# AndreiBarsan/DynSLAM

Measured on AMD Instinct MI355X. Metric: frames/sec TSDF integrate+raycast (KITTI 1242x375, 5mm voxels); HBM GB/s vs peak, higher is better.
Workload: dtype f32; 1 GPU; configs[1]: static map only, synthetic KITTI-like street 1242x375, preset 5mm (voxel 0.005 m, mu 0.02 m), frames 5..2062 of a 2063-frame sequence, one volume per GPU; visible_blocks_last_frame=122661, allocated_blocks=8388608, status=3, decay=False, swap=False, instances=0

## Files before the change

dynslam_amd/csrc/dsr_device.h:

```cpp
#pragma once
#include <hip/hip_runtime.h>
#include <stdint.h>

#include "../../include/dsr.h"

namespace dsr {

constexpr int kBlockSize = DSR_BLOCK_SIZE;
constexpr int kBlockSize3 = DSR_BLOCK_SIZE3;
constexpr int kBlockBytes = 4096;

constexpr int kOffSdf = 0;
constexpr int kOffWDepth = 1024;
constexpr int kOffClr = 2048;

constexpr float kFarAway = 999999.9f;
constexpr float kVeryClose = 0.05f;
constexpr int kMinmaxSubsample = 8;

enum Ctr {
  CTR_LAST_FREE_BLOCK = 0,
  CTR_LAST_FREE_EXCESS = 1,
  CTR_NO_VISIBLE_LIVE = 2,
  CTR_NO_VISIBLE_FREE = 3,
// ... 31 lines not shown
  Mat4 M_rgb;
  float4 proj;
  float4 proj_rgb;
  float mu, voxelSize;
  float vfMin, vfMax;
  int W, H, Wr, Hr;
  int maxW, stopAtMaxW, depthWeighting, rgbSame;
  int noBuckets, noExcess, noTotalEntries, noBlocks;
  uint32_t hashMask;
  uint32_t maxSteps;
  int useSwapping;
};

struct SceneP {
  dsr_hash_entry *table;
  uint8_t *vba;
  int32_t *voxelAllocList;
  int32_t *excessAllocList;
  int32_t *ctr;
  unsigned long long *work;
  uint32_t *allocKey;
  uint32_t *allocGrp;
  unsigned long long *allocTile;
  uint8_t *swapState;
  uint8_t *swapStored;
  int32_t *swapSlot;
  uint8_t **hostSlabs;
  int slabBlocks;
  uint8_t *visGrp;
  uint32_t *visBits;
  uint32_t *allocBits;
  int32_t *allocIds;
  float *icpPose;
};
constexpr int kIcpPoseWords = 20;
__device__ __forceinline__ void write_icp_pose(const SceneP &s, const Mat4 &M) {
  if (blockIdx.x == 0 && blockIdx.y == 0 && threadIdx.x < 17) s.icpPose[threadIdx.x] = threadIdx.x < 16 ? M.m[threadIdx.x] : 1.0f;
}


__device__ __forceinline__ int f2i(float f) {
  int r;
  asm("v_cvt_i32_f32 %0, %1" : "=v"(r) : "v"(f));
  return r;
}
__device__ __forceinline__ short f2s(float f) { return (short)f2i(f); }
// ... 68 lines not shown
template <int NT>
__device__ __forceinline__ int2 wg_exclusive_scan2(int2 v, int2 &total, int2 *lds) {
  const int lane = threadIdx.x & 63, wid = threadIdx.x >> 6;
  int2 inc = v;
#pragma unroll
  for (int d = 1; d < 64; d <<= 1) {
    int ox = __shfl_up(inc.x, d), oy = __shfl_up(inc.y, d);
    if (lane >= d) { inc.x += ox; inc.y += oy; }
  }
  if (lane == 63) lds[wid] = inc;
  __syncthreads();
  int2 woff = make_int2(0, 0), tot = make_int2(0, 0);
#pragma unroll
  for (int w = 0; w < NT / 64; ++w) {
    int2 s = lds[w];
    if (w < wid) { woff.x += s.x; woff.y += s.y; }
    tot.x += s.x; tot.y += s.y;
  }
  __syncthreads();
  total = tot;
  return make_int2(woff.x + inc.x - v.x, woff.y + inc.y - v.y);
}

constexpr int kTileThreads = 256;
constexpr int kTileItems = 8;
constexpr int kTile = kTileThreads * kTileItems;

}
```

dynslam_amd/csrc/dsr_engine.hip:

```cpp
#include <sched.h>

#include "dsr_internal.h"
#include "dsr_math.h"
using namespace dsr_internal;
#include "k_alloc.h"
#include "k_composite.h"
#include "k_decay.h"
#include "k_integrate.h"
#include "k_raycast.h"
#include "k_swap.h"
#include "k_mesh.h"
#include "k_small.h"
#include "k_batch.h"
#include "k_batch_gc.h"
#include "../../include/dsr_track.h"
#include "../../include/dsr_gc.h"

extern "C" {
int dsri_batch_flush(dsr_batch *b);
bool dsri_batch_is_live(dsr_batch *b);
void dsri_batch_drop_deferred(dsr_batch *b);
}

namespace dsr_internal {
// ... 67 lines not shown
}

int reset_scene(dsr_engine *e) {
  e->sceneVersion++;
  e->noVisibleValid = false;
  e->listVersion++;
  LAUNCH(e, "reset", k_reset_table, dim3(div_up(e->E, 256)), dim3(256), e->scene.table, e->E, e->scene.allocKey);
  LAUNCH(e, "reset", k_iota, dim3(div_up(e->noExcess, 256)), dim3(256), e->scene.excessAllocList, e->noExcess);
  LAUNCH(e, "reset", k_iota, dim3(div_up(e->noBlocks, 256)), dim3(256), e->scene.voxelAllocList, e->noBlocks);
  LAUNCH(e, "reset", k_reset_vba, dim3(4096), dim3(256), reinterpret_cast<uint4 *>(e->scene.vba),
         (size_t)e->noBlocks * (kBlockBytes / 16));
  LAUNCH(e, "reset", k_reset_counters, dim3(1), dim3(64), e->scene.ctr, e->scene.work, e->noBlocks, e->noExcess);
  if (e->scene.swapState) {
    HIP_TRY(hipMemsetAsync(e->scene.swapState, 0, (size_t)e->E, e->stream));
    HIP_TRY(hipMemsetAsync(e->scene.swapStored, 0, (size_t)e->E, e->stream));
    HIP_TRY(hipMemsetAsync(e->scene.swapSlot, 0xff, (size_t)e->E * 4, e->stream));
    HIP_TRY(hipStreamSynchronize(e->stream));
    e->hostUsedUpper = 0; e->hostUsedPending = false; e->hostUsedCallsSince = 0;
  }
  HIP_TRY(hipMemsetAsync(e->live.visType, 0, (size_t)e->E, e->stream));
  HIP_TRY(hipMemsetAsync(e->freeview.visType, 0, (size_t)e->E, e->stream));
  HIP_TRY(hipMemsetAsync(e->scene.allocGrp, 0, (size_t)e->numTilesE * (kTile / 32) * 4, e->stream));
  HIP_TRY(hipMemsetAsync(e->scene.allocTile, 0, ((size_t)e->numTilesE + 1) * 8, e->stream));
  if (e->scene.visBits) {
    HIP_TRY(hipMemsetAsync(e->scene.visGrp, 0, (size_t)kSmallBitWords * 4, e->stream));
    HIP_TRY(hipMemsetAsync(e->scene.visBits, 0, (size_t)kSmallBitWords * 4, e->stream));
    HIP_TRY(hipMemsetAsync(e->scene.allocBits, 0, (size_t)kSmallBitWords * 4, e->stream));
  }
  e->fifoHead = 0; e->fifoLen = 0;
  for (RenderStateDev *rs : {&e->live, &e->freeview})
    if (rs->rayBox) {
      hipLaunchKernelGGL(k_raybox_reset, dim3(1), dim3(RB_WORDS), 0, e->stream, rs->rayBox, (e->W + 7) / 8, (e->H + 7) / 8, e->rayBoxLive ? 1 : 0);
    }
  e->rayBoxLive = true;
  HIP_TRY(hipGetLastError());
  if (e->statusHost) {
    HIP_TRY(hipStreamSynchronize(e->stream));
    e->statusHost[0] = 0; e->statusHost[1] = DSR_OK;
  }
  return DSR_OK;
}

void free_all(dsr_engine *e) {
  auto F = [](void *p) { if (p) (void)hipFree(p); };
  F(e->scene.table); F(e->scene.vba); F(e->scene.voxelAllocList); F(e->scene.excessAllocList);
  F(e->scene.ctr); F(e->scene.icpPose); F(e->scene.work); F(e->scene.allocKey); F(e->scene.allocGrp); F(e->scene.allocTile);
  F(e->scene.visGrp); F(e->scene.visBits); F(e->scene.allocBits); F(e->scene.allocIds);
  for (RenderStateDev *rs : {&e->live, &e->freeview}) {
    F(rs->visibleIDs); F(rs->visibleIDsAlt); F(rs->visBlocks); F(rs->visBlocksAlt); F(rs->visType); F(rs->minmax); F(rs->raycastResult); F(rs->raycastImage); F(rs->rayBox);
  }
  dsr_internal::tracker_free(e);
  F(e->tileSums); F(e->integrateStats); F(e->allocList); F(e->allocWork); F(e->meshTris); F(e->rgb); F(e->depth); F(e->depthTmp); F(e->rawDepth); F(e->pointsMap); F(e->normalsMap);
  F(e->freeDepth); F(e->aosScratch);
  F(e->fifoPlanes); F(e->decayCand); F(e->decayFlags);
  if (e->maskHost) (void)hipHostFree(e->maskHost);
  for (auto ev : e->maskEvent) if (ev) (void)hipEventDestroy(ev);
  F(e->scene.swapState); F(e->scene.swapStored); F(e->swapStagingDev); F(e->swapIdsDev); F(e->swapFlagsDev);
  F(e->scene.swapSlot); F(e->scene.hostSlabs);
  if (e->hostUsedSeen) (void)hipHostFree(e->hostUsedSeen);
  if (e->hostUsedEvent) (void)hipEventDestroy(e->hostUsedEvent);
  for (auto p : e->hostSlabs) (void)hipHostFree(p);
  for (int k = 0; k < 2; ++k) {
    if (e->upPin[k]) (void)hipHostFree(e->upPin[k]);
    if (e->upSlotFree[k]) (void)hipEventDestroy(e->upSlotFree[k]);
  }
  F(e->upDev); F(e->pvDev); F(e->xferRgb); F(e->xferDepth);
  F(e->rgbAlt); F(e->depthAlt);
  for (hipEvent_t ev : {e->evAltFree, e->evFusionRead}) if (ev) (void)hipEventDestroy(ev);
  if (e->viewStream && e->ownsViewStream) (void)hipStreamDestroy(e->viewStream);
  if (e->pvPin) (void)hipHostFree(e->pvPin);
  if (e->statusHost) (void)hipHostFree(e->statusHost);
  for (hipEvent_t ev : {e->evUploaded, e->evIngested, e->evView, e->evViewRead}) if (ev) (void)hipEventDestroy(ev);
  if (e->xEvent) (void)hipEventDestroy(e->xEvent);
  if (e->xEvent2) (void)hipEventDestroy(e->xEvent2);
  if (e->orderEvent) (void)hipEventDestroy(e->orderEvent);
// ... 17 lines not shown
  { int st = before_fusion(e); if (st) return st; }
  if (e->sidePending) { HIP_TRY(hipStreamWaitEvent(e->stream, e->evExpected, 0)); e->sidePending = false; }
  if (e->smallPath) {
    const int tx0 = e->viewBox[0] / 16, ty0 = e->viewBox[1] / 16;
    const int tx1 = div_up(std::min(e->viewBox[2], e->W), 16), ty1 = div_up(std::min(e->viewBox[3], e->H), 16);
    if (tx1 > tx0 && ty1 > ty0)
      LAUNCH(e, "alloc_mark", k_alloc_mark<true>, dim3(tx1 - tx0, ty1 - ty0), dim3(256), p, e->scene, (const float *)e->depth,
             rs.visType, tx0, ty0);
    if (e->statusDev) e->statusSeq++;
    {
      ProfScope _ps(e, "small_alloc_visible");
      hipLaunchKernelGGL(k_small_alloc_visible, dim3(1), dim3(kSmallThreads), e->smallLdsBytes, e->stream, p, e->scene,
                         (const float *)e->depth, rs.visType, e->numTilesE, e->allocWork, rs.visibleIDs, rs.visBlocks, e->noBlocks,
                         e->statusDev, e->statusSeq, reinterpret_cast<int2 *>(rs.minmax), rs.rayBox, e->smallLists ? 1 : 0);
    }
    HIP_TRY(hipGetLastError());
    { int st = after_fusion(e); if (st) return st; }
    e->liveExp.valid = true; e->liveExp.onSide = false; e->liveExp.version = e->listVersion; e->liveExp.M = e->M_d;
    memcpy(e->liveExp.proj, proj, sizeof proj);
    return DSR_OK;
  }
  LAUNCH(e, "retest_prev_visible", k_retest_previous_visible, dim3(1024), dim3(256), p, e->scene,
         (const int4 *)rs.visBlocks, rs.visType);
  int2 *allocTile = reinterpret_cast<int2 *>(e->scene.allocTile);
  LAUNCH(e, "alloc_mark", k_alloc_mark<false>, dim3(div_up(e->W, 16), div_up(e->H, 16)), dim3(256), p, e->scene,
         (const float *)e->depth, rs.visType, 0, 0);
  LAUNCH(e, "scan_tiles", k_scan_tile_sums, dim3(1), dim3(1024), allocTile, e->numTilesE, e->scene, (int)SCAN_ALLOC, 0);
  LAUNCH(e, "alloc_commit", k_alloc_commit, dim3(e->numTilesE), dim3(kTileThreads), p, e->scene, allocTile, e->allocWork);
  LAUNCH(e, "alloc_apply", k_alloc_apply, dim3(256), dim3(256), p, e->scene, (const float *)e->depth,
         (const int4 *)e->allocWork, rs.visType);
  LAUNCH(e, "visible_count", k_visible_count<false>, dim3(e->numTilesE), dim3(kTileThreads), p, e->scene, rs.visType, e->tileSums);
  LAUNCH(e, "scan_tiles", k_scan_tile_sums, dim3(1), dim3(1024), e->tileSums, e->numTilesE, e->scene,
         (int)SCAN_VISIBLE_LIVE, e->noBlocks);
  if (e->statusDev) e->statusSeq++;
  LAUNCH(e, "visible_write", k_visible_write, dim3(e->numTilesE), dim3(kTileThreads), e->E, (const uint8_t *)rs.visType,
         (const int2 *)e->tileSums, rs.visibleIDs, e->noBlocks, e->scene, (int)e->s.use_swapping, rs.visBlocks, e->statusDev,
         e->statusSeq);
  HIP_TRY(hipGetLastError());
  { int st = after_fusion(e); if (st) return st; }
  e->liveExp.valid = false;
  if (e->overlapExpected && (e->device >= 64 || g_enginesOnDevice[e->device].load(std::memory_order_relaxed) <= 1)) {
    HIP_TRY(hipEventRecord(e->evList, e->stream));
    HIP_TRY(hipStreamWaitEvent(e->sideStream, e->evList, 0));
    {
      StreamSwap sw(e, e->sideStream);
      int st = expected_depths(e, rs, p);
      if (st) return st;
    }
    HIP_TRY(hipEventRecord(e->evExpected, e->sideStream));
    e->sidePending = true;
    e->liveExp.valid = true; e->liveExp.onSide = true; e->liveExp.version = e->listVersion; e->liveExp.M = e->M_d;
    memcpy(e->liveExp.proj, proj, sizeof proj);
  }
  return DSR_OK;
}

int integrate_scene(dsr_engine *e) {
  e->sceneVersion++;
  float proj[4]; depth_proj(e, proj);
  FrameP p = make_frame_params(e, e->M_d, e->invM_d, proj);
// ... 270 lines not shown
    if (e->device < 0 || e->device >= 64) return nullptr;
    std::lock_guard<std::mutex> lock(g_ioMutex);
    if (!table[e->device] && create_stream(&table[e->device]) != hipSuccess) table[e->device] = nullptr;
    return table[e->device];
  };
  if (pvMode == 3 && s.sdf_local_block_num <= 16384 && (e->stream = shared_stream(g_sharedViewStream))) e->ownsStream = false;
  else if (pvMode >= 2 && s.sdf_local_block_num <= 16384 && (e->stream = shared_stream(g_sharedSmallStream))) e->ownsStream = false;
  else if (create_stream(&e->stream) != hipSuccess) { delete e; return fail(DSR_E_DEVICE, "hipStreamCreate failed"); }
  e->overlapExpected = s.sdf_local_block_num >= (1 << 20);
  if (const char *ov = getenv("DSR_OVERLAP_EXPECTED")) e->overlapExpected = atoi(ov) != 0;
  if (e->overlapExpected &&
      (hipStreamCreateWithFlags(&e->sideStream, hipStreamNonBlocking) != hipSuccess ||
       hipEventCreateWithFlags(&e->evList, order_event_flags()) != hipSuccess ||
       hipEventCreateWithFlags(&e->evExpected, order_event_flags()) != hipSuccess)) { free_all(e); delete e; return fail(DSR_E_DEVICE, "side stream creation failed"); }
  ALLOC(dmalloc(&e->scene.table, (size_t)e->E));
  ALLOC(dmalloc(&e->scene.vba, (size_t)e->noBlocks * kBlockBytes));
  ALLOC(dmalloc(&e->scene.voxelAllocList, (size_t)e->noBlocks));
  ALLOC(dmalloc(&e->scene.excessAllocList, (size_t)e->noExcess));
  ALLOC(dmalloc(&e->scene.ctr, (size_t)CTR_COUNT));
  ALLOC(dmalloc(&e->scene.work, (size_t)WORK_COUNT));
  ALLOC(dmalloc(&e->scene.allocKey, (size_t)e->E));
  ALLOC(dmalloc(&e->scene.allocGrp, (size_t)e->numTilesE * (kTile / 32)));
  ALLOC(dmalloc(&e->scene.allocTile, (size_t)e->numTilesE + 1));
  {
    const int cells = ((e->W + 7) / 8) * ((e->H + 7) / 8);
    e->smallPath = e->smallVolume && !s.use_swapping && e->E <= kSmallMaxEntries && e->E % 8 == 0 && e->numTilesE <= kSmallMaxTiles &&
                   small_lds_bytes(cells) <= 64 * 1024;
    if (e->smallPath) {
      ALLOC(dmalloc(&e->scene.visGrp, (size_t)kSmallBitWords * 4));
      ALLOC(dmalloc(&e->scene.visBits, (size_t)kSmallBitWords));
      ALLOC(dmalloc(&e->scene.allocBits, (size_t)kSmallBitWords));
      ALLOC(dmalloc(&e->scene.allocIds, (size_t)e->noBlocks));
      e->smallLdsBytes = small_lds_bytes(cells);
      const size_t withLists = std::max(e->smallLdsBytes, sizeof(SmallShared) + small_lists_lds_bytes(e->noBlocks));
      e->smallLists = withLists <= 64 * 1024 && !(getenv("DSR_SMALL_LISTS") && atoi(getenv("DSR_SMALL_LISTS")) == 0);
      if (e->smallLists) e->smallLdsBytes = withLists;
      e->pairRender = pair_render_default();
    }
  }
  ALLOC(dmalloc(&e->allocWork, (size_t)std::min((double)e->noBlocks, (double)e->P * e->maxSteps)));
  const int mw = (e->W + 7) / 8, mh = (e->H + 7) / 8;
  for (RenderStateDev *rs : {&e->live, &e->freeview}) {
    ALLOC(dmalloc(&rs->visibleIDs, (size_t)e->noBlocks));
    ALLOC(dmalloc(&rs->visBlocks, (size_t)e->noBlocks));
    ALLOC(dmalloc(&rs->visType, (size_t)e->E));
    ALLOC(dmalloc(&rs->minmax, (size_t)mw * mh));
// ... 390 lines not shown
        break;
      }
      if (!cached && e->smallPath) {
        const int cells = ((e->W + 7) / 8) * ((e->H + 7) / 8);
        {
          ProfScope _ps(e, "small_freeview");
          hipLaunchKernelGGL(k_small_freeview, dim3(1), dim3(kSmallThreads), small_lds_bytes(cells), e->stream, p, e->scene, e->allocList,
                             rs.visibleIDs, rs.visBlocks, e->noBlocks, reinterpret_cast<int2 *>(rs.minmax), rs.rayBox, e->smallLists ? 1 : 0);
        }
        e->fvValid = true; e->fvVersion = e->sceneVersion; e->fvM = M; memcpy(e->fvProj, proj, sizeof proj);
        if (outIsDevice) {
          LAUNCH(e, "raycast_freeview", k_raycast_render, g, dim3(256), p, e->scene, (const float2 *)rs.minmax,
                 rs.raycastResult, type, rs.raycastImage, (float *)depth_out, (uchar4 *)rgba_out, rs.rayBox);
          HIP_TRY(hipGetLastError());
          break;
        }
        LAUNCH(e, "raycast_freeview", k_raycast_render, g, dim3(256), p, e->scene, (const float2 *)rs.minmax,
               rs.raycastResult, type, rs.raycastImage, depth_out ? e->freeDepth : (float *)nullptr, (uchar4 *)nullptr, rs.rayBox);
        HIP_TRY(hipGetLastError());
        if (rgba_out) HIP_TRY(hipMemcpyAsync(rgba_out, rs.raycastImage, P * 4, kind, e->stream));
        if (depth_out) HIP_TRY(hipMemcpyAsync(depth_out, e->freeDepth, P * 4, kind, e->stream));
        break;
      } else if (!cached && e->smallVolume) {
        LAUNCH(e, "freeview_visible", k_visible_count<true>, dim3(e->numTilesE), dim3(kTileThreads), p, e->scene, rs.visType, e->tileSums);
        LAUNCH(e, "scan_tiles", k_scan_tile_sums, dim3(1), dim3(1024), e->tileSums, e->numTilesE, e->scene,
               (int)SCAN_VISIBLE_FREE, e->noBlocks);
        LAUNCH(e, "freeview_visible", k_visible_write, dim3(e->numTilesE), dim3(kTileThreads), e->E, (const uint8_t *)rs.visType,
               (const int2 *)e->tileSums, rs.visibleIDs, e->noBlocks, e->scene, 0, rs.visBlocks, (int32_t *)nullptr, 0);
        int st = expected_depths(e, rs, p);
        if (st) return st;
        e->fvValid = true; e->fvVersion = e->sceneVersion; e->fvM = M; memcpy(e->fvProj, proj, sizeof proj);
        if (outIsDevice) {
          LAUNCH(e, "raycast_freeview", k_raycast_render, g, dim3(256), p, e->scene, (const float2 *)rs.minmax,
                 rs.raycastResult, type, rs.raycastImage, (float *)depth_out, (uchar4 *)rgba_out, rs.rayBox);
          HIP_TRY(hipGetLastError());
          break;
        }
        LAUNCH(e, "raycast_freeview", k_raycast_render, g, dim3(256), p, e->scene, (const float2 *)rs.minmax,
               rs.raycastResult, type, rs.raycastImage, depth_out ? e->freeDepth : (float *)nullptr, (uchar4 *)nullptr, rs.rayBox);
        HIP_TRY(hipGetLastError());
        if (rgba_out) HIP_TRY(hipMemcpyAsync(rgba_out, rs.raycastImage, P * 4, kind, e->stream));
        if (depth_out) HIP_TRY(hipMemcpyAsync(depth_out, e->freeDepth, P * 4, kind, e->stream));
        break;
      } else if (!cached) {
      if (e->allocListVersion != e->sceneVersion) {
        LAUNCH(e, "allocated_list", k_allocated_count, dim3(e->numTilesE), dim3(kTileThreads), e->scene, e->E, e->tileSums);
        LAUNCH(e, "scan_tiles", k_scan_tile_sums, dim3(1), dim3(1024), e->tileSums, e->numTilesE, e->scene,
               (int)SCAN_ALLOCATED, e->noBlocks);
        LAUNCH(e, "allocated_list", k_allocated_write, dim3(e->numTilesE), dim3(kTileThreads), e->scene, e->E,
               (const int2 *)e->tileSums, e->allocList, e->noBlocks);
        e->allocListVersion = e->sceneVersion;
// ... 760 lines not shown
```

dynslam_amd/csrc/dsr_internal.h:

```cpp
#pragma once
#include <hip/hip_runtime.h>

#include <algorithm>
#include <atomic>
#include <cmath>
#include <cstdio>
#include <cstdlib>
#include <cstring>
#include <map>
#include <mutex>
#include <new>
#include <string>
#include <unordered_map>
#include <vector>

#include "dsr_device.h"
#include "../../include/dsr_track.h"

using namespace dsr;

namespace dsr_internal {
std::string &last_error();
inline int fail(int code, const std::string &msg) { last_error() = msg; return code; }
}
// ... 34 lines not shown
  bool overlapExpected = true;
  unsigned long long listVersion = 0;
  struct { bool valid = false; bool onSide = false; unsigned long long version = 0; Mat4 M; float proj[4] = {0, 0, 0, 0}; } liveExp;
  int W = 0, H = 0, Wr = 0, Hr = 0, P = 0;
  int noBuckets = 0, noExcess = 0, E = 0, noBlocks = 0;
  int numTilesE = 0, numTilesB = 0, numTilesMax = 0;
  uint32_t maxSteps = 0;
  int gridPersistent = 2048;
  int gridDecay = 2048;
  int gridIntegrate = 8192;
  bool smallVolume = false;
  bool smallPath = false;
  bool smallLists = false;
  size_t smallLdsBytes = 0;
  int viewBox[4] = {0, 0, 0, 0};
  int blankBox[4] = {0, 0, 0, 0};
  bool blankValid = false;
  int gridExpected = 128;
  Mat4 calibInv, M_d, invM_d;

  SceneP scene{};
  RenderStateDev live, freeview;
  int2 *tileSums = nullptr;
  uint2 *integrateStats = nullptr;
  size_t integrateStatsCount = 0;
  int4 *allocWork = nullptr;
  unsigned long long sceneVersion = 0;
  int32_t *allocList = nullptr;
  unsigned long long allocListVersion = ~0ull;
  bool fvValid = false;
  unsigned long long fvVersion = 0;
  Mat4 fvM;
  float fvProj[4] = {0, 0, 0, 0};
  dsr_triangle *meshTris = nullptr;
  uint64_t meshCount = 0;

  bool hasView = false;
  uchar4 *rgb = nullptr;
  float *depth = nullptr, *depthTmp = nullptr;
  short *rawDepth = nullptr;
  float4 *pointsMap = nullptr, *normalsMap = nullptr;
  float *freeDepth = nullptr;
  dsr_voxel *aosScratch = nullptr;
  int aosScratchBlocks = 0;

  int depthWeighting = 0;
// ... 168 lines not shown
```

dynslam_amd/csrc/k_alloc.h:

```cpp
#pragma once
#include "dsr_device.h"

namespace dsr {


struct AllocRay {
  float px, py, pz;
  float dx, dy, dz;
  int noSteps;
};

template <class Ops = DeviceOps>
__host__ __device__ __forceinline__ bool alloc_ray(const FrameP &p, const float *__restrict__ depth, int x, int y, AllocRay &r) {
  float depth_measure = depth[x + y * p.W];
  if (depth_measure <= 0 || (depth_measure - p.mu) < 0 || (depth_measure - p.mu) < p.vfMin ||
      (depth_measure + p.mu) > p.vfMax)
    return false;
  const float oneOverVoxelSize = 1.0f / (p.voxelSize * (float)kBlockSize);
  const float invFx = 1.0f / p.proj.x, invFy = 1.0f / p.proj.y;
  float cz = depth_measure;
  float cx = cz * (((float)x - p.proj.z) * invFx);
  float cy = cz * (((float)y - p.proj.w) * invFy);
  float norm = Ops::sqrt(cx * cx + cy * cy + cz * cz);
  float f1 = 1.0f - p.mu / norm;
  float3 t = mat_mul3(p.invM, cx * f1, cy * f1, cz * f1, 1.0f);
  r.px = t.x * oneOverVoxelSize; r.py = t.y * oneOverVoxelSize; r.pz = t.z * oneOverVoxelSize;
  float f2 = 1.0f + p.mu / norm;
  t = mat_mul3(p.invM, cx * f2, cy * f2, cz * f2, 1.0f);
  float ex = t.x * oneOverVoxelSize, ey = t.y * oneOverVoxelSize, ez = t.z * oneOverVoxelSize;
  float dx = ex - r.px, dy = ey - r.py, dz = ez - r.pz;
  norm = Ops::sqrt(dx * dx + dy * dy + dz * dz);
  r.noSteps = Ops::f2i(Ops::ceil(2.0f * norm));
  float denom = (float)(r.noSteps - 1);
  r.dx = dx / denom; r.dy = dy / denom; r.dz = dz / denom;
  return true;
}

constexpr uint8_t kTouchedNow = 0x81;
template <bool BITS>
__device__ __forceinline__ void alloc_mark_pixel(const FrameP &p, const SceneP &s, const float *__restrict__ depth,
                                                 uint8_t *__restrict__ visType, int x, int y, bool inImage) {
  AllocRay r;
  r.px = r.py = r.pz = r.dx = r.dy = r.dz = 0.0f; r.noSteps = 0;
  bool ok = inImage && alloc_ray(p, depth, x, y, r);
  if (ok && (uint32_t)(r.noSteps > 0 ? r.noSteps : 0) > p.maxSteps) {
    s.ctr[CTR_STATUS] = DSR_E_ARG;
    ok = false;
  }
  const int noSteps = ok ? r.noSteps : 0;
  int waveSteps = noSteps;
  if (BITS) {
#pragma unroll
    for (int d = 1; d < 64; d <<= 1) { const int o = __shfl_xor(waveSteps, d); waveSteps = o > waveSteps ? o : waveSteps; }
  }
  const int lane = threadIdx.x & 63;
  const uint32_t keyBase = (uint32_t)(x + y * p.W) * p.maxSteps + 1u;
  float px = r.px, py = r.py, pz = r.pz;
  for (int i0 = 0; i0 < waveSteps; i0 += 4) {
    short cb[4][3];
    uint32_t ch[4];
// ... 49 lines not shown
    bool covered[4] = {false, false, false, false};
    if (BITS) {
      const bool hasRight = (lane & 15) != 15, hasBelow = lane < 48;
#pragma unroll
      for (int kk = 0; kk < 4; ++kk) {
        const uint32_t right = (uint32_t)__shfl_down((int)tgt[kk], 1), below = (uint32_t)__shfl_down((int)tgt[kk], 16);
#pragma unroll
        for (int k = 0; k < 4; ++k) {
          if (hasRight && right == tgt[k]) covered[k] = true;
          if (hasBelow && below == tgt[k]) covered[k] = true;
          if (kk > k && tgt[kk] == tgt[k]) covered[k] = true;
        }
      }
    }
    uint32_t old[4] = {1u, 1u, 1u, 1u};
#pragma unroll
    for (int k = 0; k < 4; ++k)
      if (tgt[k] != kNoTarget && !covered[k]) old[k] = atomicMax(&s.allocKey[tgt[k]], keyBase + (uint32_t)(i0 + k));
#pragma unroll
    for (int k = 0; k < 4; ++k) {
      if (tgt[k] != kNoTarget && !covered[k] && old[k] == 0u) {
        const uint32_t one = exc[k] ? 0x11u : 0x01u;
        atomicAdd(&s.allocGrp[tgt[k] >> 5], one << (((tgt[k] >> 3) & 3u) * 8u));
        atomicAdd(&s.allocTile[tgt[k] / (uint32_t)kTile], exc[k] ? 0x100000001ull : 1ull);
      }
    }
  }
}

__device__ __forceinline__ void alloc_winner_pos(const FrameP &p, const float *__restrict__ depth, uint32_t key,
                                                 short &bx, short &by, short &bz) {
  const uint32_t k = key - 1u;
  const uint32_t pixel = k / p.maxSteps, step = k - pixel * p.maxSteps;
  const int y = (int)(pixel / (uint32_t)p.W), x = (int)(pixel - (uint32_t)y * (uint32_t)p.W);
  AllocRay r;
  alloc_ray(p, depth, x, y, r);
  float px = r.px, py = r.py, pz = r.pz;
  for (uint32_t i = 0; i < step; ++i) { px += r.dx; py += r.dy; pz += r.dz; }
  bx = f2s(floorf(px)); by = f2s(floorf(py)); bz = f2s(floorf(pz));
}

enum ScanMode { SCAN_ALLOC = 0, SCAN_VISIBLE_LIVE = 1, SCAN_VISIBLE_FREE = 2, SCAN_DECAY = 3, SCAN_COMPACT_LIVE = 4, SCAN_NCAND = 5, SCAN_SWAP_IN = 6, SCAN_SWAP_OUT = 7, SCAN_MESH = 8, SCAN_ALLOCATED = 9 };
template <int NT>
__device__ __forceinline__ void scan_tile_sums_body(int2 *__restrict__ tileSums, int numTiles, const SceneP &s, int mode,
                                                    int capacity, int2 *lds) {
  int2 carry = make_int2(0, 0);
  constexpr int kPer = 8;
  if (numTiles <= NT * kPer) {
    const int base = threadIdx.x * kPer;
    int2 v[kPer];
    int2 sum = make_int2(0, 0);
#pragma unroll
    for (int j = 0; j < kPer; ++j) {
      v[j] = (base + j < numTiles) ? tileSums[base + j] : make_int2(0, 0);
      sum.x += v[j].x; sum.y += v[j].y;
    }
    int2 run = wg_exclusive_scan2<NT>(sum, carry, lds);
#pragma unroll
    for (int j = 0; j < kPer; ++j) {
      if (base + j < numTiles) tileSums[base + j] = run;
      run.x += v[j].x; run.y += v[j].y;
    }
  } else {
    for (int base = 0; base < numTiles; base += NT) {
      int i = base + threadIdx.x;
      int2 v = (i < numTiles) ? tileSums[i] : make_int2(0, 0);
      int2 total;
      int2 ex = wg_exclusive_scan2<NT>(v, total, lds);
      if (i < numTiles) tileSums[i] = make_int2(carry.x + ex.x, carry.y + ex.y);
      carry.x += total.x; carry.y += total.y;
    }
  }
  if (threadIdx.x == 0) {
    int32_t *ctr = s.ctr;
    if (mode == SCAN_ALLOC) {
      const int oldV = ctr[CTR_LAST_FREE_BLOCK], oldE = ctr[CTR_LAST_FREE_EXCESS];
      ctr[CTR_ALLOC_OLD_HEAD_VBA] = oldV; ctr[CTR_ALLOC_OLD_HEAD_EXC] = oldE;
      ctr[CTR_ALLOC_TOTAL12] = carry.x; ctr[CTR_ALLOC_TOTAL2] = carry.y;
      int nv = oldV - carry.x, ne = oldE - carry.y;
      ctr[CTR_LAST_FREE_BLOCK] = nv < -1 ? -1 : nv;
      ctr[CTR_LAST_FREE_EXCESS] = ne < -1 ? -1 : ne;
      if (carry.x > oldV + 1 || carry.y > oldE + 1) ctr[CTR_STATUS] = DSR_E_OUT_OF_BLOCKS;
    } else if (mode == SCAN_VISIBLE_LIVE || mode == SCAN_VISIBLE_FREE || mode == SCAN_COMPACT_LIVE) {
      int n = carry.x < capacity ? carry.x : capacity;
      if (mode == SCAN_COMPACT_LIVE) ctr[CTR_TMP_OLD_NVIS] = ctr[CTR_NO_VISIBLE_LIVE];
      ctr[mode == SCAN_VISIBLE_FREE ? CTR_NO_VISIBLE_FREE : CTR_NO_VISIBLE_LIVE] = n;
      if (mode == SCAN_VISIBLE_LIVE) {
        ctr[CTR_VIS_OVERFLOW] = carry.x > capacity ? 1 : 0;
        const int oldV = ctr[CTR_LAST_FREE_BLOCK];
        ctr[CTR_ALLOC_OLD_HEAD_VBA] = oldV;
        const int nv = oldV - carry.y;
        ctr[CTR_LAST_FREE_BLOCK] = nv < -1 ? -1 : nv;
        if (carry.y > oldV + 1) ctr[CTR_STATUS] = DSR_E_OUT_OF_BLOCKS;
      }
    } else if (mode == SCAN_SWAP_IN || mode == SCAN_SWAP_OUT) {
      const int n = carry.x < capacity ? carry.x : capacity;
      ctr[CTR_SWAP_COUNT] = n;
      if (mode == SCAN_SWAP_OUT) {
        ctr[CTR_ALLOC_OLD_HEAD_VBA] = ctr[CTR_LAST_FREE_BLOCK];
        ctr[CTR_LAST_FREE_BLOCK] += n;
        ctr[CTR_SWAP_FIRST_SLOT] = ctr[CTR_HOST_USED];
      }
    } else if (mode == SCAN_ALLOCATED) {
      ctr[CTR_NO_ALLOCATED] = carry.x < capacity ? carry.x : capacity;
    } else if (mode == SCAN_MESH) {
      ctr[CTR_MESH_TOTAL] = carry.x;
    } else if (mode == SCAN_NCAND) {
      ctr[CTR_DECAY_NCAND] = carry.x < capacity ? carry.x : capacity;
    } else if (mode == SCAN_DECAY) {
      ctr[CTR_DECAY_FREED] = carry.x;
      ctr[CTR_ALLOC_OLD_HEAD_VBA] = ctr[CTR_LAST_FREE_BLOCK];
      ctr[CTR_LAST_FREE_BLOCK] += carry.x;
      atomicAdd(&s.work[WORK_DECAYED_BLOCKS], (unsigned long long)carry.x);
    }
  }
}
__global__ __launch_bounds__(1024) void k_scan_tile_sums(int2 *__restrict__ tileSums, int numTiles, SceneP s, int mode,
                                                         int capacity) {
  __shared__ int2 lds[1024 / 64];
  scan_tile_sums_body<1024>(tileSums, numTiles, s, mode, capacity, lds);
}


template <bool BITS>
__global__ __launch_bounds__(256) void k_alloc_mark(FrameP p, SceneP s, const float *__restrict__ depth,
                                                    uint8_t *__restrict__ visType, int tileX0, int tileY0) {
  const int x = (blockIdx.x + tileX0) * 16 + (threadIdx.x & 15), y = (blockIdx.y + tileY0) * 16 + (threadIdx.x >> 4);
  alloc_mark_pixel<BITS>(p, s, depth, visType, x, y, x < p.W && y < p.H);
}

__global__ __launch_bounds__(kTileThreads) void k_alloc_commit(FrameP p, SceneP s, int2 *__restrict__ tileOffsets,
                                                               int4 *__restrict__ workList) {
  __shared__ int2 lds[kTileThreads / 64];
  const int base = blockIdx.x * kTile + threadIdx.x * kTileItems;
  uint32_t *grpWord = s.allocGrp + (base >> 5);
  const uint32_t word = (base < p.noTotalEntries) ? *grpWord : 0u;
  const uint32_t byte = (word >> (((base >> 3) & 3) * 8)) & 0xffu;
  const int2 c = make_int2((int)(byte & 15u), (int)(byte >> 4));
  if (word != 0u && (threadIdx.x & 3) == 0) *grpWord = 0u;
  const int2 tileOff = tileOffsets[blockIdx.x];
  int2 total;
  int2 ex = wg_exclusive_scan2<kTileThreads>(c, total, lds);
  if (threadIdx.x == 0) tileOffsets[blockIdx.x] = make_int2(0, 0);
  if (c.x == 0) return;
  int rank12 = tileOff.x + ex.x, rank2 = tileOff.y + ex.y;
  const int oldV = s.ctr[CTR_ALLOC_OLD_HEAD_VBA], oldE = s.ctr[CTR_ALLOC_OLD_HEAD_EXC];
  uint32_t key[kTileItems];
  int ptrOf[kTileItems];
#pragma unroll
  for (int j = 0; j < kTileItems; ++j) {
    const int t = base + j < p.noTotalEntries ? base + j : p.noTotalEntries - 1;
    key[j] = s.allocKey[t];
    ptrOf[j] = s.table[t].ptr;
  }
#pragma unroll
  for (int j = 0; j < kTileItems; ++j)
    if (base + j >= p.noTotalEntries) key[j] = 0u;
#pragma unroll
  for (int j = 0; j < kTileItems; ++j) {
    const int t = base + j;
    const uint32_t k = key[j];
    if (!k) continue;
    const bool isExc = ptrOf[j] >= -1;
    s.allocKey[t] = 0u;
    const int vbaIdx = oldV - rank12;
    int exlIdx = 0;
    if (isExc) { exlIdx = oldE - rank2; rank2++; }
    if (vbaIdx >= 0) workList[rank12] = make_int4(exlIdx >= 0 ? t : -1, (int)k, vbaIdx, isExc ? exlIdx : -1);
    rank12++;
// ... 8 lines not shown
  short bx, by, bz;
  alloc_winner_pos(p, depth, (uint32_t)w.y, bx, by, bz);
  const int px = (int)((uint32_t)(uint16_t)bx | ((uint32_t)(uint16_t)by << 16));
  const int pz = (int)(uint32_t)(uint16_t)bz;
  const int ptr = s.voxelAllocList[w.z];
  if (w.w < 0) {
    dsr_hash_entry *he = s.table + t;
    *reinterpret_cast<int2 *>(he) = make_int2(px, pz);
    he->ptr = ptr;
    if (BITS) atomicOr(&s.allocBits[t >> 5], 1u << (t & 31));
  } else {
    const int exlOffset = s.excessAllocList[w.w];
    s.table[t].offset = exlOffset + 1;
    const int child = p.noBuckets + exlOffset;
    *reinterpret_cast<int4 *>(s.table + child) = make_int4(px, pz, 0, ptr);
    visType[child] = (BITS && lists) ? kTouchedNow : (uint8_t)1;
    if (BITS) {
      if (!lists) atomicOr(&s.visBits[child >> 5], 1u << (child & 31));
      atomicOr(&s.allocBits[child >> 5], 1u << (child & 31));
    }
  }
}
__global__ __launch_bounds__(256) void k_alloc_apply(FrameP p, SceneP s, const float *__restrict__ depth,
                                                     const int4 *__restrict__ workList, uint8_t *__restrict__ visType) {
  const int total = s.ctr[CTR_ALLOC_TOTAL12], avail = s.ctr[CTR_ALLOC_OLD_HEAD_VBA] + 1;
  const int n = total < avail ? total : avail;
  for (int i = blockIdx.x * blockDim.x + threadIdx.x; i < n; i += gridDim.x * blockDim.x)
    alloc_apply_item<false>(p, s, depth, workList[i], visType);
}


template <bool useSwapping, class Ops = DeviceOps>
__host__ __device__ __forceinline__ void check_point_visibility(bool &isVisible, bool &isVisibleEnlarged, float x, float y, float z,
                                                                const Mat4 &M, const float4 &proj, int W, int H) {
  float3 b = mat_mul3(M, x, y, z, 1.0f);
  if (b.z < 1e-10f) return;
  const float yz = Ops::rcp(b.z);
  float u = Ops::div(proj.x * b.x, b.z, yz) + proj.z;
  float v = Ops::div(proj.y * b.y, b.z, yz) + proj.w;
  if (u >= 0 && u < (float)W && v >= 0 && v < (float)H) {
    isVisible = true; isVisibleEnlarged = true;
  } else if (useSwapping) {
    int lx = -W / 8, ly = W + W / 8, lz = -H / 8, lw = H + H / 8;
    if (u >= (float)lx && u < (float)ly && v >= (float)lz && v < (float)lw) isVisibleEnlarged = true;
  }
}
template <bool useSwapping, class Ops = DeviceOps>
__host__ __device__ __forceinline__ void check_block_visibility(bool &isVisible, bool &isVisibleEnlarged, const short pos[3],
                                                                const Mat4 &M, const float4 &proj, float voxelSize, int W, int H) {
// ... 30 lines not shown
    } else {
      check_block_visibility<false>(isVisible, isVisibleEnlarged, he.pos, p.M, p.proj, p.voxelSize, p.W, p.H);
      visType[t] = isVisible ? 3 : 0;
    }
  }
  if (s.ctr[CTR_VIS_OVERFLOW]) {
    for (int t = blockIdx.x * blockDim.x + threadIdx.x; t < p.noTotalEntries; t += gridDim.x * blockDim.x) {
      if (visType[t] != 3) continue;
      const dsr_hash_entry he = load_entry(s.table, t);
      bool isVisible, isVisibleEnlarged;
      if (p.useSwapping) {
        check_block_visibility<true>(isVisible, isVisibleEnlarged, he.pos, p.M, p.proj, p.voxelSize, p.W, p.H);
        if (!isVisibleEnlarged) visType[t] = 0;
      } else {
        check_block_visibility<false>(isVisible, isVisibleEnlarged, he.pos, p.M, p.proj, p.voxelSize, p.W, p.H);
        if (!isVisible) visType[t] = 0;
      }
    }
  }
}

template <bool FREEVIEW>
__global__ __launch_bounds__(kTileThreads) void k_visible_count(FrameP p, SceneP s, uint8_t *__restrict__ visType,
                                                                int2 *__restrict__ tileSums) {
  __shared__ int2 lds[kTileThreads / 64];
  const int base = blockIdx.x * kTile + threadIdx.x * kTileItems;
  int2 c = make_int2(0, 0);
  uint8_t v[kTileItems];
  if (!FREEVIEW) {
    if (base + kTileItems <= p.noTotalEntries) {
      uint2 raw = *reinterpret_cast<const uint2 *>(visType + base);
#pragma unroll
      for (int j = 0; j < 4; ++j) { v[j] = (raw.x >> (8 * j)) & 0xff; v[4 + j] = (raw.y >> (8 * j)) & 0xff; }
    } else {
#pragma unroll
      for (int j = 0; j < kTileItems; ++j) v[j] = (base + j < p.noTotalEntries) ? visType[base + j] : 0;
    }
  }
#pragma unroll
  for (int j = 0; j < kTileItems; ++j) {
    const int t = base + j;
    if (FREEVIEW) {
      uint8_t vis = 0;
      if (t < p.noTotalEntries) {
        dsr_hash_entry he = load_entry(s.table, t);
        if (he.ptr >= 0) {
          bool isVisible, isVisibleEnlarged;
          check_block_visibility<false>(isVisible, isVisibleEnlarged, he.pos, p.M, p.proj, p.voxelSize, p.W, p.H);
          vis = isVisible ? 1 : 0;
        }
        visType[t] = vis;
      }
      if (vis) c.x++;
    } else {
      if (v[j] > 0) {
        c.x++;
        if (p.useSwapping) {
          if (s.swapState[t] != 2) s.swapState[t] = 1;
          if (s.table[t].ptr == -1) c.y++;
        }
      }
    }
  }
  int2 total;
  wg_exclusive_scan2<kTileThreads>(c, total, lds);
  if (threadIdx.x == 0) tileSums[blockIdx.x] = total;
}

__global__ __launch_bounds__(kTileThreads) void k_visible_write(int noTotalEntries, const uint8_t *__restrict__ visType,
                                                                const int2 *__restrict__ tileOffsets,
                                                                int32_t *__restrict__ visibleIDs, int capacity,
                                                                SceneP s, int useSwapping, int4 *__restrict__ visBlocks,
                                                                int32_t *__restrict__ publish, int publishSeq) {
  __shared__ int2 lds[kTileThreads / 64];
  if (publish && blockIdx.x == 0 && threadIdx.x == 0) {
    publish[0] = s.ctr[CTR_NO_VISIBLE_LIVE];
    publish[1] = s.ctr[CTR_STATUS];
    __hip_atomic_store(publish + 2, publishSeq, __ATOMIC_RELEASE, __HIP_MEMORY_SCOPE_SYSTEM);
  }
  const int base = blockIdx.x * kTile + threadIdx.x * kTileItems;
  uint8_t v[kTileItems];
  bool re[kTileItems];
  int2 c = make_int2(0, 0);
#pragma unroll
  for (int j = 0; j < kTileItems; ++j) {
    v[j] = (base + j < noTotalEntries) ? visType[base + j] : 0;
    re[j] = false;
    if (v[j] > 0) {
      c.x++;
      if (useSwapping && s.table[base + j].ptr == -1) { re[j] = true; c.y++; }
    }
  }
  int4 rawE[kTileItems];
#pragma unroll
  for (int j = 0; j < kTileItems; ++j) {
    rawE[j] = make_int4(0, 0, 0, -2);
    if (v[j] > 0) rawE[j] = *reinterpret_cast<const int4 *>(s.table + (base + j));
  }
  int2 total;
  int2 ex = wg_exclusive_scan2<kTileThreads>(c, total, lds);
  if (total.x == 0) return;
  const int2 off = tileOffsets[blockIdx.x];
  int rank = off.x + ex.x, rrank = off.y + ex.y;
  const int oldHead = useSwapping ? s.ctr[CTR_ALLOC_OLD_HEAD_VBA] : 0;
#pragma unroll
  for (int j = 0; j < kTileItems; ++j)
    if (v[j] > 0) {
      int4 raw = rawE[j];
      if (re[j]) {
        const int vbaIdx = oldHead - rrank;
        rrank++;
        if (vbaIdx >= 0) { raw.w = s.voxelAllocList[vbaIdx]; s.table[base + j].ptr = raw.w; }
      }
      if (rank < capacity) { visibleIDs[rank] = base + j; visBlocks[rank] = make_vis_record(raw, base + j); }
      rank++;
    }
}

}
```

Baseline: 3773 frames/s.

## Replace single-block tile scans with coarse atomic sums and in-kernel offsets

Removes the two single-workgroup k_scan_tile_sums launches (alloc and visible) from the per-frame fusion path. Per-tile counts are now also accumulated atomically into coarse 64-tile groups. Each consuming block then computes its own exclusive offset by summing its coarse prefix and the fine tiles inside its group. Counter bookkeeping (free-list heads, totals, overflow, status publish) moves into the last block of commit/write and into alloc_apply and visible_count. The cost is extra atomics and redundant per-block prefix reads, and it relies on the last-block-launched ordering for counter updates.

```diff
diff --git a/dynslam_amd/csrc/dsr_device.h b/dynslam_amd/csrc/dsr_device.h
--- a/dynslam_amd/csrc/dsr_device.h
+++ b/dynslam_amd/csrc/dsr_device.h
@@ -77,6 +77,7 @@
   uint32_t *allocKey;
   uint32_t *allocGrp;
   unsigned long long *allocTile;
+  unsigned long long *allocCoarse;
   uint8_t *swapState;
   uint8_t *swapStored;
   int32_t *swapSlot;
@@ -191,6 +192,31 @@
   return make_int2(woff.x + inc.x - v.x, woff.y + inc.y - v.y);
 }
 
+template <int NT>
+__device__ __forceinline__ int2 wg_exclusive_scan2_sum2(int2 v, int2 w, int2 &total, int2 &wsum, int4 *lds) {
+  const int lane = threadIdx.x & 63, wid = threadIdx.x >> 6;
+  int2 inc = v;
+#pragma unroll
+  for (int d = 1; d < 64; d <<= 1) {
+    int ox = __shfl_up(inc.x, d), oy = __shfl_up(inc.y, d);
+    if (lane >= d) { inc.x += ox; inc.y += oy; }
+    w.x += __shfl_xor(w.x, d); w.y += __shfl_xor(w.y, d);
+  }
+  if (lane == 63) lds[wid] = make_int4(inc.x, inc.y, w.x, w.y);
+  __syncthreads();
+  int2 woff = make_int2(0, 0), tot = make_int2(0, 0), ws = make_int2(0, 0);
+#pragma unroll
+  for (int k = 0; k < NT / 64; ++k) {
+    int4 s = lds[k];
+    if (k < wid) { woff.x += s.x; woff.y += s.y; }
+    tot.x += s.x; tot.y += s.y;
+    ws.x += s.z; ws.y += s.w;
+  }
+  __syncthreads();
+  total = tot; wsum = ws;
+  return make_int2(woff.x + inc.x - v.x, woff.y + inc.y - v.y);
+}
+
 constexpr int kTileThreads = 256;
 constexpr int kTileItems = 8;
 constexpr int kTile = kTileThreads * kTileItems;
diff --git a/dynslam_amd/csrc/dsr_engine.hip b/dynslam_amd/csrc/dsr_engine.hip
--- a/dynslam_amd/csrc/dsr_engine.hip
+++ b/dynslam_amd/csrc/dsr_engine.hip
@@ -113,6 +113,8 @@
   HIP_TRY(hipMemsetAsync(e->freeview.visType, 0, (size_t)e->E, e->stream));
   HIP_TRY(hipMemsetAsync(e->scene.allocGrp, 0, (size_t)e->numTilesE * (kTile / 32) * 4, e->stream));
   HIP_TRY(hipMemsetAsync(e->scene.allocTile, 0, ((size_t)e->numTilesE + 1) * 8, e->stream));
+  HIP_TRY(hipMemsetAsync(e->scene.allocCoarse, 0, (size_t)div_up(e->numTilesE, kCoarseTiles) * 8, e->stream));
+  HIP_TRY(hipMemsetAsync(e->visCoarse, 0, (size_t)div_up(e->numTilesE, kCoarseTiles) * 8, e->stream));
   if (e->scene.visBits) {
     HIP_TRY(hipMemsetAsync(e->scene.visGrp, 0, (size_t)kSmallBitWords * 4, e->stream));
     HIP_TRY(hipMemsetAsync(e->scene.visBits, 0, (size_t)kSmallBitWords * 4, e->stream));
@@ -135,13 +137,13 @@
 void free_all(dsr_engine *e) {
   auto F = [](void *p) { if (p) (void)hipFree(p); };
   F(e->scene.table); F(e->scene.vba); F(e->scene.voxelAllocList); F(e->scene.excessAllocList);
-  F(e->scene.ctr); F(e->scene.icpPose); F(e->scene.work); F(e->scene.allocKey); F(e->scene.allocGrp); F(e->scene.allocTile);
+  F(e->scene.ctr); F(e->scene.icpPose); F(e->scene.work); F(e->scene.allocKey); F(e->scene.allocGrp); F(e->scene.allocTile); F(e->scene.allocCoarse);
   F(e->scene.visGrp); F(e->scene.visBits); F(e->scene.allocBits); F(e->scene.allocIds);
   for (RenderStateDev *rs : {&e->live, &e->freeview}) {
     F(rs->visibleIDs); F(rs->visibleIDsAlt); F(rs->visBlocks); F(rs->visBlocksAlt); F(rs->visType); F(rs->minmax); F(rs->raycastResult); F(rs->raycastImage); F(rs->rayBox);
   }
   dsr_internal::tracker_free(e);
-  F(e->tileSums); F(e->integrateStats); F(e->allocList); F(e->allocWork); F(e->meshTris); F(e->rgb); F(e->depth); F(e->depthTmp); F(e->rawDepth); F(e->pointsMap); F(e->normalsMap);
+  F(e->tileSums); F(e->visCoarse); F(e->integrateStats); F(e->allocList); F(e->allocWork); F(e->meshTris); F(e->rgb); F(e->depth); F(e->depthTmp); F(e->rawDepth); F(e->pointsMap); F(e->normalsMap);
   F(e->freeDepth); F(e->aosScratch);
   F(e->fifoPlanes); F(e->decayCand); F(e->decayFlags);
   if (e->maskHost) (void)hipHostFree(e->maskHost);
@@ -205,20 +207,17 @@
   }
   LAUNCH(e, "retest_prev_visible", k_retest_previous_visible, dim3(1024), dim3(256), p, e->scene,
          (const int4 *)rs.visBlocks, rs.visType);
-  int2 *allocTile = reinterpret_cast<int2 *>(e->scene.allocTile);
   LAUNCH(e, "alloc_mark", k_alloc_mark<false>, dim3(div_up(e->W, 16), div_up(e->H, 16)), dim3(256), p, e->scene,
          (const float *)e->depth, rs.visType, 0, 0);
-  LAUNCH(e, "scan_tiles", k_scan_tile_sums, dim3(1), dim3(1024), allocTile, e->numTilesE, e->scene, (int)SCAN_ALLOC, 0);
-  LAUNCH(e, "alloc_commit", k_alloc_commit, dim3(e->numTilesE), dim3(kTileThreads), p, e->scene, allocTile, e->allocWork);
+  LAUNCH(e, "alloc_commit", k_alloc_commit, dim3(e->numTilesE), dim3(kTileThreads), p, e->scene, e->allocWork);
   LAUNCH(e, "alloc_apply", k_alloc_apply, dim3(256), dim3(256), p, e->scene, (const float *)e->depth,
-         (const int4 *)e->allocWork, rs.visType);
-  LAUNCH(e, "visible_count", k_visible_count<false>, dim3(e->numTilesE), dim3(kTileThreads), p, e->scene, rs.visType, e->tileSums);
-  LAUNCH(e, "scan_tiles", k_scan_tile_sums, dim3(1), dim3(1024), e->tileSums, e->numTilesE, e->scene,
-         (int)SCAN_VISIBLE_LIVE, e->noBlocks);
+         (const int4 *)e->allocWork, rs.visType, e->numTilesE, e->visCoarse);
+  LAUNCH(e, "visible_count", k_visible_count<false>, dim3(e->numTilesE), dim3(kTileThreads), p, e->scene, rs.visType, e->tileSums,
+         e->visCoarse);
   if (e->statusDev) e->statusSeq++;
-  LAUNCH(e, "visible_write", k_visible_write, dim3(e->numTilesE), dim3(kTileThreads), e->E, (const uint8_t *)rs.visType,
-         (const int2 *)e->tileSums, rs.visibleIDs, e->noBlocks, e->scene, (int)e->s.use_swapping, rs.visBlocks, e->statusDev,
-         e->statusSeq);
+  LAUNCH(e, "visible_write", k_visible_write<true>, dim3(e->numTilesE), dim3(kTileThreads), e->E, (const uint8_t *)rs.visType,
+         (const int2 *)e->tileSums, reinterpret_cast<const int2 *>(e->visCoarse), rs.visibleIDs, e->noBlocks, e->scene,
+         (int)e->s.use_swapping, rs.visBlocks, e->statusDev, e->statusSeq);
   HIP_TRY(hipGetLastError());
   { int st = after_fusion(e); if (st) return st; }
   e->liveExp.valid = false;
@@ -535,6 +534,8 @@
   ALLOC(dmalloc(&e->scene.allocKey, (size_t)e->E));
   ALLOC(dmalloc(&e->scene.allocGrp, (size_t)e->numTilesE * (kTile / 32)));
   ALLOC(dmalloc(&e->scene.allocTile, (size_t)e->numTilesE + 1));
+  ALLOC(dmalloc(&e->scene.allocCoarse, (size_t)div_up(e->numTilesE, kCoarseTiles)));
+  ALLOC(dmalloc(&e->visCoarse, (size_t)div_up(e->numTilesE, kCoarseTiles)));
   {
     const int cells = ((e->W + 7) / 8) * ((e->H + 7) / 8);
     e->smallPath = e->smallVolume && !s.use_swapping && e->E <= kSmallMaxEntries && e->E % 8 == 0 && e->numTilesE <= kSmallMaxTiles &&
@@ -971,11 +972,13 @@
         if (depth_out) HIP_TRY(hipMemcpyAsync(depth_out, e->freeDepth, P * 4, kind, e->stream));
         break;
       } else if (!cached && e->smallVolume) {
-        LAUNCH(e, "freeview_visible", k_visible_count<true>, dim3(e->numTilesE), dim3(kTileThreads), p, e->scene, rs.visType, e->tileSums);
+        LAUNCH(e, "freeview_visible", k_visible_count<true>, dim3(e->numTilesE), dim3(kTileThreads), p, e->scene, rs.visType, e->tileSums,
+               (unsigned long long *)nullptr);
         LAUNCH(e, "scan_tiles", k_scan_tile_sums, dim3(1), dim3(1024), e->tileSums, e->numTilesE, e->scene,
                (int)SCAN_VISIBLE_FREE, e->noBlocks);
-        LAUNCH(e, "freeview_visible", k_visible_write, dim3(e->numTilesE), dim3(kTileThreads), e->E, (const uint8_t *)rs.visType,
-               (const int2 *)e->tileSums, rs.visibleIDs, e->noBlocks, e->scene, 0, rs.visBlocks, (int32_t *)nullptr, 0);
+        LAUNCH(e, "freeview_visible", k_visible_write<false>, dim3(e->numTilesE), dim3(kTileThreads), e->E, (const uint8_t *)rs.visType,
+               (const int2 *)e->tileSums, (const int2 *)nullptr, rs.visibleIDs, e->noBlocks, e->scene, 0, rs.visBlocks,
+               (int32_t *)nullptr, 0);
         int st = expected_depths(e, rs, p);
         if (st) return st;
         e->fvValid = true; e->fvVersion = e->sceneVersion; e->fvM = M; memcpy(e->fvProj, proj, sizeof proj);
diff --git a/dynslam_amd/csrc/dsr_internal.h b/dynslam_amd/csrc/dsr_internal.h
--- a/dynslam_amd/csrc/dsr_internal.h
+++ b/dynslam_amd/csrc/dsr_internal.h
@@ -80,6 +80,7 @@
   SceneP scene{};
   RenderStateDev live, freeview;
   int2 *tileSums = nullptr;
+  unsigned long long *visCoarse = nullptr;
   uint2 *integrateStats = nullptr;
   size_t integrateStatsCount = 0;
   int4 *allocWork = nullptr;
diff --git a/dynslam_amd/csrc/k_alloc.h b/dynslam_amd/csrc/k_alloc.h
--- a/dynslam_amd/csrc/k_alloc.h
+++ b/dynslam_amd/csrc/k_alloc.h
@@ -36,6 +36,17 @@
   return true;
 }
 
+constexpr int kCoarseTiles = 64;
+template <class Ops = DeviceOps>
+__host__ __device__ __forceinline__ int2 tile_offset_part(const int2 *__restrict__ coarse, const int2 *__restrict__ fine, int tile,
+                                                          int tid, int nt) {
+  const int g = tile / kCoarseTiles, r = tile - g * kCoarseTiles;
+  int2 part = make_int2(0, 0);
+  for (int j = tid; j < r; j += nt) { const int2 v = fine[g * kCoarseTiles + j]; part.x += v.x; part.y += v.y; }
+  for (int i = (tid + nt - kCoarseTiles % nt) % nt; i < g; i += nt) { const int2 v = coarse[i]; part.x += v.x; part.y += v.y; }
+  return part;
+}
+
 constexpr uint8_t kTouchedNow = 0x81;
 template <bool BITS>
 __device__ __forceinline__ void alloc_mark_pixel(const FrameP &p, const SceneP &s, const float *__restrict__ depth,
@@ -131,7 +142,9 @@
       if (tgt[k] != kNoTarget && !covered[k] && old[k] == 0u) {
         const uint32_t one = exc[k] ? 0x11u : 0x01u;
         atomicAdd(&s.allocGrp[tgt[k] >> 5], one << (((tgt[k] >> 3) & 3u) * 8u));
-        atomicAdd(&s.allocTile[tgt[k] / (uint32_t)kTile], exc[k] ? 0x100000001ull : 1ull);
+        const uint32_t tile = tgt[k] / (uint32_t)kTile;
+        atomicAdd(&s.allocTile[tile], exc[k] ? 0x100000001ull : 1ull);
+        if (!BITS) atomicAdd(&s.allocCoarse[tile / (uint32_t)kCoarseTiles], exc[k] ? 0x100000001ull : 1ull);
       }
     }
   }
@@ -149,7 +162,7 @@
   bx = f2s(floorf(px)); by = f2s(floorf(py)); bz = f2s(floorf(pz));
 }
 
-enum ScanMode { SCAN_ALLOC = 0, SCAN_VISIBLE_LIVE = 1, SCAN_VISIBLE_FREE = 2, SCAN_DECAY = 3, SCAN_COMPACT_LIVE = 4, SCAN_NCAND = 5, SCAN_SWAP_IN = 6, SCAN_SWAP_OUT = 7, SCAN_MESH = 8, SCAN_ALLOCATED = 9 };
+enum ScanMode { SCAN_VISIBLE_FREE = 2, SCAN_DECAY = 3, SCAN_COMPACT_LIVE = 4, SCAN_NCAND = 5, SCAN_SWAP_IN = 6, SCAN_SWAP_OUT = 7, SCAN_MESH = 8, SCAN_ALLOCATED = 9 };
 template <int NT>
 __device__ __forceinline__ void scan_tile_sums_body(int2 *__restrict__ tileSums, int numTiles, const SceneP &s, int mode,
                                                     int capacity, int2 *lds) {
@@ -182,26 +195,10 @@
   }
   if (threadIdx.x == 0) {
     int32_t *ctr = s.ctr;
-    if (mode == SCAN_ALLOC) {
-      const int oldV = ctr[CTR_LAST_FREE_BLOCK], oldE = ctr[CTR_LAST_FREE_EXCESS];
-      ctr[CTR_ALLOC_OLD_HEAD_VBA] = oldV; ctr[CTR_ALLOC_OLD_HEAD_EXC] = oldE;
-      ctr[CTR_ALLOC_TOTAL12] = carry.x; ctr[CTR_ALLOC_TOTAL2] = carry.y;
-      int nv = oldV - carry.x, ne = oldE - carry.y;
-      ctr[CTR_LAST_FREE_BLOCK] = nv < -1 ? -1 : nv;
-      ctr[CTR_LAST_FREE_EXCESS] = ne < -1 ? -1 : ne;
-      if (carry.x > oldV + 1 || carry.y > oldE + 1) ctr[CTR_STATUS] = DSR_E_OUT_OF_BLOCKS;
-    } else if (mode == SCAN_VISIBLE_LIVE || mode == SCAN_VISIBLE_FREE || mode == SCAN_COMPACT_LIVE) {
+    if (mode == SCAN_VISIBLE_FREE || mode == SCAN_COMPACT_LIVE) {
       int n = carry.x < capacity ? carry.x : capacity;
       if (mode == SCAN_COMPACT_LIVE) ctr[CTR_TMP_OLD_NVIS] = ctr[CTR_NO_VISIBLE_LIVE];
       ctr[mode == SCAN_VISIBLE_FREE ? CTR_NO_VISIBLE_FREE : CTR_NO_VISIBLE_LIVE] = n;
-      if (mode == SCAN_VISIBLE_LIVE) {
-        ctr[CTR_VIS_OVERFLOW] = carry.x > capacity ? 1 : 0;
-        const int oldV = ctr[CTR_LAST_FREE_BLOCK];
-        ctr[CTR_ALLOC_OLD_HEAD_VBA] = oldV;
-        const int nv = oldV - carry.y;
-        ctr[CTR_LAST_FREE_BLOCK] = nv < -1 ? -1 : nv;
-        if (carry.y > oldV + 1) ctr[CTR_STATUS] = DSR_E_OUT_OF_BLOCKS;
-      }
     } else if (mode == SCAN_SWAP_IN || mode == SCAN_SWAP_OUT) {
       const int n = carry.x < capacity ? carry.x : capacity;
       ctr[CTR_SWAP_COUNT] = n;
@@ -238,22 +235,28 @@
   alloc_mark_pixel<BITS>(p, s, depth, visType, x, y, x < p.W && y < p.H);
 }
 
-__global__ __launch_bounds__(kTileThreads) void k_alloc_commit(FrameP p, SceneP s, int2 *__restrict__ tileOffsets,
-                                                               int4 *__restrict__ workList) {
-  __shared__ int2 lds[kTileThreads / 64];
+__global__ __launch_bounds__(kTileThreads) void k_alloc_commit(FrameP p, SceneP s, int4 *__restrict__ workList) {
+  __shared__ int4 lds[kTileThreads / 64];
   const int base = blockIdx.x * kTile + threadIdx.x * kTileItems;
   uint32_t *grpWord = s.allocGrp + (base >> 5);
   const uint32_t word = (base < p.noTotalEntries) ? *grpWord : 0u;
   const uint32_t byte = (word >> (((base >> 3) & 3) * 8)) & 0xffu;
   const int2 c = make_int2((int)(byte & 15u), (int)(byte >> 4));
   if (word != 0u && (threadIdx.x & 3) == 0) *grpWord = 0u;
-  const int2 tileOff = tileOffsets[blockIdx.x];
-  int2 total;
-  int2 ex = wg_exclusive_scan2<kTileThreads>(c, total, lds);
-  if (threadIdx.x == 0) tileOffsets[blockIdx.x] = make_int2(0, 0);
+  const int2 part = tile_offset_part(reinterpret_cast<const int2 *>(s.allocCoarse), reinterpret_cast<const int2 *>(s.allocTile),
+                                     (int)blockIdx.x, (int)threadIdx.x, kTileThreads);
+  const int oldV = s.ctr[CTR_LAST_FREE_BLOCK], oldE = s.ctr[CTR_LAST_FREE_EXCESS];
+  int2 total, tileOff;
+  int2 ex = wg_exclusive_scan2_sum2<kTileThreads>(c, part, total, tileOff, lds);
+  if (blockIdx.x == gridDim.x - 1 && threadIdx.x == 0) {
+    const int all12 = tileOff.x + total.x, all2 = tileOff.y + total.y;
+    int32_t *ctr = s.ctr;
+    ctr[CTR_ALLOC_OLD_HEAD_VBA] = oldV; ctr[CTR_ALLOC_OLD_HEAD_EXC] = oldE;
+    ctr[CTR_ALLOC_TOTAL12] = all12; ctr[CTR_ALLOC_TOTAL2] = all2;
+    if (all12 > oldV + 1 || all2 > oldE + 1) ctr[CTR_STATUS] = DSR_E_OUT_OF_BLOCKS;
+  }
   if (c.x == 0) return;
   int rank12 = tileOff.x + ex.x, rank2 = tileOff.y + ex.y;
-  const int oldV = s.ctr[CTR_ALLOC_OLD_HEAD_VBA], oldE = s.ctr[CTR_ALLOC_OLD_HEAD_EXC];
   uint32_t key[kTileItems];
   int ptrOf[kTileItems];
 #pragma unroll
@@ -308,9 +311,19 @@
   }
 }
 __global__ __launch_bounds__(256) void k_alloc_apply(FrameP p, SceneP s, const float *__restrict__ depth,
-                                                     const int4 *__restrict__ workList, uint8_t *__restrict__ visType) {
+                                                     const int4 *__restrict__ workList, uint8_t *__restrict__ visType, int numTiles,
+                                                     unsigned long long *__restrict__ visCoarse) {
   const int total = s.ctr[CTR_ALLOC_TOTAL12], avail = s.ctr[CTR_ALLOC_OLD_HEAD_VBA] + 1;
   const int n = total < avail ? total : avail;
+  const int gtid = blockIdx.x * blockDim.x + threadIdx.x;
+  if (gtid == 0) {
+    const int nv = avail - 1 - total, ne = s.ctr[CTR_ALLOC_OLD_HEAD_EXC] - s.ctr[CTR_ALLOC_TOTAL2];
+    s.ctr[CTR_LAST_FREE_BLOCK] = nv < -1 ? -1 : nv;
+    s.ctr[CTR_LAST_FREE_EXCESS] = ne < -1 ? -1 : ne;
+  }
+  const int numCoarse = (numTiles + kCoarseTiles - 1) / kCoarseTiles;
+  for (int i = gtid; i < numTiles; i += gridDim.x * blockDim.x) s.allocTile[i] = 0ull;
+  for (int i = gtid; i < numCoarse; i += gridDim.x * blockDim.x) { s.allocCoarse[i] = 0ull; visCoarse[i] = 0ull; }
   for (int i = blockIdx.x * blockDim.x + threadIdx.x; i < n; i += gridDim.x * blockDim.x)
     alloc_apply_item<false>(p, s, depth, workList[i], visType);
 }
@@ -387,7 +400,7 @@
 
 template <bool FREEVIEW>
 __global__ __launch_bounds__(kTileThreads) void k_visible_count(FrameP p, SceneP s, uint8_t *__restrict__ visType,
-                                                                int2 *__restrict__ tileSums) {
+                                                                int2 *__restrict__ tileSums, unsigned long long *__restrict__ coarse) {
   __shared__ int2 lds[kTileThreads / 64];
   const int base = blockIdx.x * kTile + threadIdx.x * kTileItems;
   int2 c = make_int2(0, 0);
@@ -429,20 +442,22 @@
   }
   int2 total;
   wg_exclusive_scan2<kTileThreads>(c, total, lds);
-  if (threadIdx.x == 0) tileSums[blockIdx.x] = total;
-}
-
+  if (threadIdx.x == 0) {
+    tileSums[blockIdx.x] = total;
+    if (!FREEVIEW) {
+      if (total.x) atomicAdd(&coarse[blockIdx.x / kCoarseTiles], (unsigned long long)(uint32_t)total.x | ((unsigned long long)(uint32_t)total.y << 32));
+      if (blockIdx.x == 0) s.ctr[CTR_ALLOC_OLD_HEAD_VBA] = s.ctr[CTR_LAST_FREE_BLOCK];
+    }
+  }
+}
+
+template <bool LIVE>
 __global__ __launch_bounds__(kTileThreads) void k_visible_write(int noTotalEntries, const uint8_t *__restrict__ visType,
-                                                                const int2 *__restrict__ tileOffsets,
+                                                                const int2 *__restrict__ tileSums, const int2 *__restrict__ coarse,
                                                                 int32_t *__restrict__ visibleIDs, int capacity,
                                                                 SceneP s, int useSwapping, int4 *__restrict__ visBlocks,
                                                                 int32_t *__restrict__ publish, int publishSeq) {
-  __shared__ int2 lds[kTileThreads / 64];
-  if (publish && blockIdx.x == 0 && threadIdx.x == 0) {
-    publish[0] = s.ctr[CTR_NO_VISIBLE_LIVE];
-    publish[1] = s.ctr[CTR_STATUS];
-    __hip_atomic_store(publish + 2, publishSeq, __ATOMIC_RELEASE, __HIP_MEMORY_SCOPE_SYSTEM);
-  }
+  __shared__ int4 lds[kTileThreads / 64];
   const int base = blockIdx.x * kTile + threadIdx.x * kTileItems;
   uint8_t v[kTileItems];
   bool re[kTileItems];
@@ -462,10 +477,35 @@
     rawE[j] = make_int4(0, 0, 0, -2);
     if (v[j] > 0) rawE[j] = *reinterpret_cast<const int4 *>(s.table + (base + j));
   }
-  int2 total;
-  int2 ex = wg_exclusive_scan2<kTileThreads>(c, total, lds);
-  if (total.x == 0) return;
-  const int2 off = tileOffsets[blockIdx.x];
+  int2 total, off, ex;
+  if (LIVE) {
+    const int2 part = tile_offset_part(coarse, tileSums, (int)blockIdx.x, (int)threadIdx.x, kTileThreads);
+    ex = wg_exclusive_scan2_sum2<kTileThreads>(c, part, total, off, lds);
+    if (blockIdx.x == gridDim.x - 1 && threadIdx.x == 0) {
+      int32_t *ctr = s.ctr;
+      const int all = off.x + total.x, allRe = off.y + total.y;
+      const int n = all < capacity ? all : capacity;
+      ctr[CTR_NO_VISIBLE_LIVE] = n;
+      ctr[CTR_VIS_OVERFLOW] = all > capacity ? 1 : 0;
+      int status = ctr[CTR_STATUS];
+      if (useSwapping) {
+        const int oldV = ctr[CTR_ALLOC_OLD_HEAD_VBA];
+        const int nv = oldV - allRe;
+        ctr[CTR_LAST_FREE_BLOCK] = nv < -1 ? -1 : nv;
+        if (allRe > oldV + 1) { status = DSR_E_OUT_OF_BLOCKS; ctr[CTR_STATUS] = status; }
+      }
+      if (publish) {
+        publish[0] = n;
+        publish[1] = status;
+        __hip_atomic_store(publish + 2, publishSeq, __ATOMIC_RELEASE, __HIP_MEMORY_SCOPE_SYSTEM);
+      }
+    }
+    if (total.x == 0) return;
+  } else {
+    ex = wg_exclusive_scan2<kTileThreads>(c, total, reinterpret_cast<int2 *>(lds));
+    if (total.x == 0) return;
+    off = tileSums[blockIdx.x];
+  }
   int rank = off.x + ex.x, rrank = off.y + ex.y;
   const int oldHead = useSwapping ? s.ctr[CTR_ALLOC_OLD_HEAD_VBA] : 0;
 #pragma unroll
```

Result: slower. 1774 frames/s (-53.0%).
